# marvinquiet/SpaDOT

Hardware: AMD Instinct MI355X
Metric: training steps/sec + Sinkhorn iters/sec, 50k spots x 3k genes x 5 timepoints (higher is better)
Workload: dtype bf16; 1 GPU; cfg3: 5 time points x 10000 spots x 3000 genes, batch 512, k=30, 1200 inducing points; parallelism=1 GPU, n_sub=9980, E_sub=308893, m_inducing=236, params=16136032, hip_graphs=True, staged_graphs=True, bucketed_grad_exchange=False, units_in_schedule=80

## Files before the change

### spadot_amd/csrc/gemm_bf16.hip

```cpp
#include <hip/hip_runtime.h>
#include <cstdint>

#include "../../include/spadot_model.h"
#include "per_device.h"

#ifndef GEMM_ABLATE
#define GEMM_ABLATE 0
#endif

namespace {

typedef __bf16 bf8 __attribute__((ext_vector_type(8)));
typedef float f16v __attribute__((ext_vector_type(16)));

constexpr int BM = 320, BN = 256, BK = 64, STAGES = 2, NT = 512;
constexpr int ROWB = BK * 2;
constexpr int STAGE_ROWS = BM + BN;
constexpr int STAGEB = STAGE_ROWS * ROWB;
constexpr int PIECES = STAGE_ROWS / 8 / 8;
constexpr int LDS_BYTES = STAGES * STAGEB;

__device__ __forceinline__ unsigned pack2(float lo, float hi) {
    const unsigned short a = __builtin_bit_cast(unsigned short, (__bf16)lo), b = __builtin_bit_cast(unsigned short, (__bf16)hi);
    return (unsigned)a | ((unsigned)b << 16);
}

typedef short s4v __attribute__((ext_vector_type(4)));

template <bool BT>
__global__ __launch_bounds__(NT, 1) void k_gemm_bf16(const __bf16 *__restrict__ A, int lda, const __bf16 *__restrict__ B,
                                                    int ldb, __bf16 *__restrict__ C, int ldc, int M, int N, int K,
                                                    int mtiles, int ntiles, int full_items, int S, int nk_slice,
                                                    float *__restrict__ part, const __bf16 *__restrict__ msk, int ldm, float slope) {
    extern __shared__ __attribute__((aligned(16))) unsigned char smem[];
    const int total = mtiles * ntiles;
    const int full_grid = 8 * ((full_items + 7) >> 3);
    int item, slice = 0;
    if ((int)blockIdx.x < full_grid) {
        const int per_xcd = (full_items + 7) >> 3;
        item = (int)(blockIdx.x & 7) * per_xcd + (int)(blockIdx.x >> 3);
        if (item >= full_items) return;
    } else {
        const int t = (int)blockIdx.x - full_grid;
        item = full_items + t / S;
        slice = t - (t / S) * S;
        if (item >= total) return;
    }
    const bool sliced = item >= full_items;
    const int ks0 = sliced ? slice * nk_slice : 0;
    const int mt = item / ntiles, nt = item - mt * ntiles;
    const int m0 = mt * BM, n0 = nt * BN;
    const int tid = threadIdx.x, lane = tid & 63;
    const int wave = __builtin_amdgcn_readfirstlane(tid >> 6);
    const int wm = wave >> 2, wn = wave & 3;
    const unsigned lds0 = (unsigned)(size_t)smem;

    unsigned off[PIECES];
#pragma unroll
    for (int u = 0; u < PIECES; u++) {
        const int row = 8 * (wave + 8 * u) + (lane >> 3);
        const int chunk = (lane & 7) ^ ((row >> 1) & 7);
        if (u < 5) {
            off[u] = (unsigned)min(m0 + row, M - 1) * (unsigned)(lda * 2) + chunk * 16;
        } else if (!BT) {
            off[u] = (unsigned)(n0 + row - BM) * (unsigned)(ldb * 2) + chunk * 16;
        } else {
            const int brow = 2 * (wave + 8 * (u - 5)) + (lane >> 5);
            off[u] = (unsigned)brow * (unsigned)(ldb * 2) + (unsigned)n0 * 2 + (((lane & 31) ^ ((brow & 3) << 2)) << 4);
        }
    }
    auto request = [&](int ks) __attribute__((always_inline)) {
        const unsigned base = lds0 + (unsigned)(ks % STAGES) * STAGEB + (unsigned)wave * 1024u;
        const char *ga = reinterpret_cast<const char *>(A) + (size_t)(ks0 + ks) * ROWB;
        const char *gb = reinterpret_cast<const char *>(B) + (BT ? (size_t)(ks0 + ks) * BK * ldb * 2 : (size_t)(ks0 + ks) * ROWB);
#pragma unroll
        for (int u = 0; u < PIECES; u++) {
            unsigned keep;
            const unsigned dst = __builtin_amdgcn_readfirstlane(base + (unsigned)u * 8192u);
            asm volatile("s_mov_b32 %0, m0\n\ts_mov_b32 m0, %3\n\ts_nop 0\n\tglobal_load_lds_dwordx4 %1, %2\n\ts_mov_b32 m0, %0"
                         : "=&s"(keep) : "v"(off[u]), "s"(u < 5 ? ga : gb), "s"(dst) : "memory");
        }
    };

    f16v acc[5][2];
#pragma unroll
    for (int i = 0; i < 5; i++)
#pragma unroll
        for (int j = 0; j < 2; j++)
#pragma unroll
            for (int e = 0; e < 16; e++) acc[i][j][e] = 0.f;

    const int r = lane & 31, hh = lane >> 5;
    unsigned a_base[4], b_base[4];
#pragma unroll
    for (int s4 = 0; s4 < 4; s4++) {
        const unsigned sw = (unsigned)(((2 * s4 + hh) ^ ((r >> 1) & 7)) << 4);
        a_base[s4] = lds0 + (unsigned)(wm * 160 + r) * ROWB + sw;
        b_base[s4] = lds0 + (unsigned)(BM + wn * 64 + r) * ROWB + sw;
    }
    unsigned bt_base[2];
    {
        const int g16 = (lane >> 4) & 1, qq = (lane & 15) >> 2, pp = lane & 3;
#pragma unroll
        for (int j = 0; j < 2; j++) {
            const int g = wn * 2 + j;
            bt_base[j] = lds0 + (unsigned)(BM * ROWB) + (unsigned)((8 * hh + qq) * 512 + (g & ~3) * 64 + ((g ^ qq) & 3) * 64 + 32 * g16 + 8 * pp);
        }
    }
    auto read_frags = [&](unsigned stage_off, int s4, bf8 (&af)[5], bf8 (&bf)[2]) __attribute__((always_inline)) {
        if (GEMM_ABLATE & 4) return;
        const unsigned pb = b_base[s4] + stage_off, pa = a_base[s4] + stage_off;
        if (BT) {
#pragma unroll
            for (int j = 0; j < 2; j++) {
                s4v lo, hi;
                const unsigned p = bt_base[j] + stage_off + (unsigned)s4 * 8192u;
                asm volatile("ds_read_b64_tr_b16 %0, %1" : "=v"(lo) : "v"(p));
                asm volatile("ds_read_b64_tr_b16 %0, %1 offset:2048" : "=v"(hi) : "v"(p));
                bf[j] = __builtin_bit_cast(bf8, __builtin_shufflevector(lo, hi, 0, 1, 2, 3, 4, 5, 6, 7));
            }
        } else {
            asm volatile("ds_read_b128 %0, %1" : "=v"(bf[0]) : "v"(pb));
            asm volatile("ds_read_b128 %0, %1 offset:4096" : "=v"(bf[1]) : "v"(pb));
        }
        asm volatile("ds_read_b128 %0, %1" : "=v"(af[0]) : "v"(pa));
        asm volatile("ds_read_b128 %0, %1 offset:4096" : "=v"(af[1]) : "v"(pa));
        asm volatile("ds_read_b128 %0, %1 offset:8192" : "=v"(af[2]) : "v"(pa));
        asm volatile("ds_read_b128 %0, %1 offset:12288" : "=v"(af[3]) : "v"(pa));
        asm volatile("ds_read_b128 %0, %1 offset:16384" : "=v"(af[4]) : "v"(pa));
    };
    auto mma = [&](const bf8 (&af)[5], const bf8 (&bf)[2]) __attribute__((always_inline)) {
        if (GEMM_ABLATE & 2) {
#pragma unroll
            for (int i = 0; i < 5; i++) asm volatile("" ::"v"(af[i]));
#pragma unroll
            for (int j = 0; j < 2; j++) asm volatile("" ::"v"(bf[j]));
            return;
        }
        __builtin_amdgcn_s_setprio(1);
#pragma unroll
        for (int i = 0; i < 5; i++)
#pragma unroll
            for (int j = 0; j < 2; j++) acc[i][j] = __builtin_amdgcn_mfma_f32_32x32x16_bf16(bf[j], af[i], acc[i][j], 0, 0, 0);
        __builtin_amdgcn_s_setprio(0);
    };
    auto frags_ready = [&]() __attribute__((always_inline)) {
        if (BT) asm volatile("s_waitcnt lgkmcnt(9)" ::: "memory");
        else asm volatile("s_waitcnt lgkmcnt(7)" ::: "memory");
        __builtin_amdgcn_sched_barrier(0);
    };

    const int nk = sliced ? min(nk_slice, K / BK - ks0) : K / BK;
    request(0);
    if (1 < nk) {
        request(1);
        asm volatile("s_waitcnt vmcnt(%0)" ::"n"(PIECES) : "memory");
    } else {
        asm volatile("s_waitcnt vmcnt(0)" ::: "memory");
    }
    __builtin_amdgcn_s_barrier();
    bf8 a0[5], b0[2], a1[5], b1[2];
    read_frags(0u, 0, a0, b0);
    for (int P = 0; P < nk; P++) {
        const unsigned so = (unsigned)(P % STAGES) * STAGEB;
        read_frags(so, 1, a1, b1);
        frags_ready();
        mma(a0, b0);
        read_frags(so, 2, a0, b0);
        frags_ready();
        mma(a1, b1);
        read_frags(so, 3, a1, b1);
        frags_ready();
        mma(a0, b0);
        if (P + 1 < nk) {
            asm volatile("s_waitcnt vmcnt(0)" ::: "memory");
            asm volatile("s_waitcnt lgkmcnt(0)" ::: "memory");
            __builtin_amdgcn_sched_barrier(0);
            __builtin_amdgcn_s_barrier();
            if (P + 2 < nk && !(GEMM_ABLATE & 1)) request(P + 2);
            read_frags((unsigned)((P + 1) % STAGES) * STAGEB, 0, a0, b0);
            if (BT) asm volatile("s_waitcnt lgkmcnt(9)" ::: "memory");
            else asm volatile("s_waitcnt lgkmcnt(7)" ::: "memory");
        } else {
            asm volatile("s_waitcnt lgkmcnt(0)" ::: "memory");
        }
        __builtin_amdgcn_sched_barrier(0);
        mma(a1, b1);
    }

    __syncthreads();
    if (sliced) {
        float *tile = part + ((size_t)(item - full_items) * S + slice) * (size_t)(BM * BN);
        unsigned char *patch = smem + (size_t)wave * 8192;
#pragma unroll
        for (int i = 0; i < 5; i++) {
#pragma unroll
            for (int j = 0; j < 2; j++)
#pragma unroll
                for (int g = 0; g < 4; g++) {
                    const int n = j * 32 + 8 * g + 4 * hh;
                    *reinterpret_cast<float4 *>(patch + r * 256 + n * 4) =
                        make_float4(acc[i][j][4 * g], acc[i][j][4 * g + 1], acc[i][j][4 * g + 2], acc[i][j][4 * g + 3]);
                }
            asm volatile("s_waitcnt lgkmcnt(0)" ::: "memory");
#pragma unroll
            for (int p = 0; p < 8; p++) {
                const int pr = p * 4 + (lane >> 4), pc = lane & 15;
                const float4 v = *reinterpret_cast<const float4 *>(patch + pr * 256 + pc * 16);
                *reinterpret_cast<float4 *>(tile + (size_t)(wm * 160 + i * 32 + pr) * BN + wn * 64 + pc * 4) = v;
            }
            asm volatile("s_waitcnt lgkmcnt(0)" ::: "memory");
        }
        return;
    }
    unsigned char *patch = smem + (size_t)wave * 4096;
    typedef unsigned u32x4 __attribute__((ext_vector_type(4)));
    const bool masked = msk != nullptr;
    const __bf16 *mbase = (masked ? msk : C) + n0 + wn * 64 + (lane & 7) * 8;
    const int mld = masked ? ldm : ldc;
    auto mask_row = [&](int i, int p) __attribute__((always_inline)) { return min(m0 + wm * 160 + i * 32 + p * 8 + (lane >> 3), M - 1); };
    u32x4 mkb[2][4];
    if (masked) {
#pragma unroll
        for (int p = 0; p < 4; p++) mkb[0][p] = *reinterpret_cast<const u32x4 *>(mbase + (size_t)mask_row(0, p) * mld);
    }
#pragma unroll
    for (int i = 0; i < 5; i++) {
        if (masked && i + 1 < 5) {
#pragma unroll
            for (int p = 0; p < 4; p++) mkb[(i + 1) & 1][p] = *reinterpret_cast<const u32x4 *>(mbase + (size_t)mask_row(i + 1, p) * mld);
        }
        __builtin_amdgcn_sched_barrier(0);
#pragma unroll
        for (int j = 0; j < 2; j++)
#pragma unroll
            for (int g = 0; g < 4; g++) {
                const int n = j * 32 + 8 * g + 4 * hh;
                *reinterpret_cast<uint2 *>(patch + r * 128 + n * 2) =
                    make_uint2(pack2(acc[i][j][4 * g], acc[i][j][4 * g + 1]), pack2(acc[i][j][4 * g + 2], acc[i][j][4 * g + 3]));
            }
        asm volatile("s_waitcnt lgkmcnt(0)" ::: "memory");
#pragma unroll
        for (int p = 0; p < 4; p++) {
            const int pr = p * 8 + (lane >> 3), pc = lane & 7;
            const int gm = m0 + wm * 160 + i * 32 + pr;
            u32x4 v = *reinterpret_cast<const u32x4 *>(patch + pr * 128 + pc * 16);
            if (masked) {
#pragma unroll
                for (int e = 0; e < 4; e++) {
                    float lo = __uint_as_float(v[e] << 16), hi = __uint_as_float(v[e] & 0xffff0000u);
                    if (!(__uint_as_float(mkb[i & 1][p][e] << 16) > 0.f)) lo *= slope;
                    if (!(__uint_as_float(mkb[i & 1][p][e] & 0xffff0000u) > 0.f)) hi *= slope;
                    v[e] = pack2(lo, hi);
                }
            }
            if (gm < M) *reinterpret_cast<u32x4 *>(C + (size_t)gm * ldc + n0 + wn * 64 + pc * 8) = v;
        }
        asm volatile("s_waitcnt lgkmcnt(0)" ::: "memory");
    }
}

__global__ __launch_bounds__(256) void k_gemm_tail_reduce(const float *__restrict__ part, int S, int ntiles, int first_mt,
                                                         __bf16 *__restrict__ C, int ldc, int M) {
    const int t = blockIdx.x / (BM / 8);
    const int row = (blockIdx.x - t * (BM / 8)) * 8 + (threadIdx.x >> 5), cg = threadIdx.x & 31;
    const int mt = first_mt + t / ntiles, nt = t - (t / ntiles) * ntiles;
    const int gm = mt * BM + row;
    if (gm >= M) return;
    const float *src = part + (size_t)t * S * (size_t)(BM * BN) + (size_t)row * BN + cg * 8;
    float4 a = *reinterpret_cast<const float4 *>(src), b = *reinterpret_cast<const float4 *>(src + 4);
    for (int s_ = 1; s_ < S; s_++) {
        const float4 c = *reinterpret_cast<const float4 *>(src + (size_t)s_ * (BM * BN));
        const float4 d = *reinterpret_cast<const float4 *>(src + (size_t)s_ * (BM * BN) + 4);
        a.x += c.x; a.y += c.y; a.z += c.z; a.w += c.w;
        b.x += d.x; b.y += d.y; b.z += d.z; b.w += d.w;
    }
    *reinterpret_cast<uint4 *>(C + (size_t)gm * ldc + nt * BN + cg * 8) =
        make_uint4(pack2(a.x, a.y), pack2(a.z, a.w), pack2(b.x, b.y), pack2(b.z, b.w));
}

}

template <bool BT>
static int launch_gemm(const void *A, int lda, const void *B, int ldb, void *C, int ldc, int M, int N, int K, void *stream,
                       const void *msk = nullptr, int ldm = 0, float slope = 1.f) {
    if (msk && (ldm < N || ldm % 8 || ((uintptr_t)msk & 15))) return -22;
    if (M <= 0 || N <= 0 || K <= 0 || N % BN != 0 || K % BK != 0 || lda < K || ldb < (BT ? N : K) || ldc < N) return -22;
    if (((uintptr_t)A & 15) || ((uintptr_t)B & 15) || ((uintptr_t)C & 15) || lda % 8 || ldb % 8 || ldc % 8) return -22;
    if ((size_t)M * lda * 2 >= ((size_t)1 << 32) || (size_t)(BT ? K : N) * ldb * 2 >= ((size_t)1 << 32)) return -22;
    static PerDeviceFlag attr_set;     
    if (!attr_set) {
        if (hipFuncSetAttribute((const void *)k_gemm_bf16<BT>, hipFuncAttributeMaxDynamicSharedMemorySize, LDS_BYTES) != hipSuccess) return -5;
        attr_set = true;
    }
    const int mtiles = (M + BM - 1) / BM, ntiles = N / BN;
    const unsigned grid = 8u * (unsigned)((mtiles * ntiles + 7) / 8);
    hipLaunchKernelGGL(k_gemm_bf16<BT>, dim3(grid), dim3(NT), LDS_BYTES, (hipStream_t)stream, (const __bf16 *)A, lda,
                       (const __bf16 *)B, ldb, (__bf16 *)C, ldc, M, N, K, mtiles, ntiles, mtiles * ntiles, 1, K / BK, (float *)nullptr,
                       (const __bf16 *)msk, ldm, slope);
    return hipGetLastError() == hipSuccess ? 0 : -5;
}

extern "C" long long spadot_gemm_bf16_split_workspace(int M, int N, int tail_row_tiles, int slices) {
    if (M <= 0 || N <= 0 || N % BN != 0 || tail_row_tiles < 1 || slices < 2 || slices > 8) return -22;
    const int mtiles = (M + BM - 1) / BM;
    if (tail_row_tiles > mtiles) return -22;
    return (long long)tail_row_tiles * (N / BN) * slices * BM * BN;
}

extern "C" int spadot_gemm_tn_bf16_split(const void *A, int lda, const void *B, int ldb, void *C, int ldc, int M, int N, int K,
                                         int tail_row_tiles, int slices, float *workspace, void *stream) {
    if (M <= 0 || N <= 0 || K <= 0 || N % BN != 0 || K % BK != 0 || lda < K || ldb < K || ldc < N) return -22;
    if (((uintptr_t)A & 15) || ((uintptr_t)B & 15) || ((uintptr_t)C & 15) || lda % 8 || ldb % 8 || ldc % 8) return -22;
    if ((size_t)M * lda * 2 >= ((size_t)1 << 32) || (size_t)N * ldb * 2 >= ((size_t)1 << 32)) return -22;
    const int mtiles = (M + BM - 1) / BM, ntiles = N / BN, nk = K / BK;
    if (tail_row_tiles < 1 || tail_row_tiles > mtiles || slices < 2 || slices > 8 || slices > nk) return -22;
    if (!workspace || ((uintptr_t)workspace & 15)) return -22;
    static PerDeviceFlag attr_set;     
    if (!attr_set) {
        if (hipFuncSetAttribute((const void *)k_gemm_bf16<false>, hipFuncAttributeMaxDynamicSharedMemorySize, LDS_BYTES) != hipSuccess) return -5;
        attr_set = true;
    }
    const int nk_slice = (nk + slices - 1) / slices;
    const int S = (nk + nk_slice - 1) / nk_slice;
    const int full_items = (mtiles - tail_row_tiles) * ntiles, tail_tiles = tail_row_tiles * ntiles;
    const unsigned grid = 8u * (unsigned)((full_items + 7) / 8) + (unsigned)(tail_tiles * S);
    hipLaunchKernelGGL(k_gemm_bf16<false>, dim3(grid), dim3(NT), LDS_BYTES, (hipStream_t)stream, (const __bf16 *)A, lda,
                       (const __bf16 *)B, ldb, (__bf16 *)C, ldc, M, N, K, mtiles, ntiles, full_items, S, nk_slice, workspace,
                       (const __bf16 *)nullptr, 0, 1.f);
    hipLaunchKernelGGL(k_gemm_tail_reduce, dim3((unsigned)(tail_tiles * (BM / 8))), dim3(256), 0, (hipStream_t)stream,
                       (const float *)workspace, S, ntiles, mtiles - tail_row_tiles, (__bf16 *)C, ldc, M);
    return hipGetLastError() == hipSuccess ? 0 : -5;
}

extern "C" int spadot_gemm_tn_bf16(const void *A, int lda, const void *B, int ldb, void *C, int ldc, int M, int N, int K,
                                   void *stream) {
    return launch_gemm<false>(A, lda, B, ldb, C, ldc, M, N, K, stream);
}

extern "C" int spadot_gemm_nn_bf16(const void *A, int lda, const void *B, int ldb, void *C, int ldc, int M, int N, int K,
                                   void *stream) {
    return launch_gemm<true>(A, lda, B, ldb, C, ldc, M, N, K, stream);
}

extern "C" int spadot_gemm_nn_bf16_masked(const void *A, int lda, const void *B, int ldb, void *C, int ldc, int M, int N, int K,
                                          const void *act_out, int ldm, double slope, void *stream) {
    if (!act_out) return -22;
    return launch_gemm<true>(A, lda, B, ldb, C, ldc, M, N, K, stream, act_out, ldm, (float)slope);
}
```

### spadot_amd/csrc/gemm_wgrad_bf16.hip

```cpp
#include <hip/hip_runtime.h>
#include <cstdint>

#include "../../include/spadot_model.h"
#include "per_device.h"

namespace {

typedef __bf16 bf8 __attribute__((ext_vector_type(8)));
typedef short s4v __attribute__((ext_vector_type(4)));
typedef float f16v __attribute__((ext_vector_type(16)));

constexpr int TN = 256, TK = 256, CH = 64, NT = 512;
constexpr int ROWB = 512;
constexpr int OPB = CH * ROWB;
constexpr int STAGEB = 2 * OPB;
constexpr int LDS_BYTES = 2 * STAGEB;
constexpr int PIECES = 8;

template <int WGN, int WGK, int TI, int TJ>
__global__ __launch_bounds__(NT, 1) void k_gemm_wgrad_bf16(const __bf16 *__restrict__ G, int ldg, const __bf16 *__restrict__ X,
                                                          int ldx, float *__restrict__ dW, int ldw, int M, int N, int K,
                                                          int ktiles, int S, int chunks_per_slice,
                                                          const __bf16 *__restrict__ zrow, float *__restrict__ part) {
    extern __shared__ __attribute__((aligned(16))) unsigned char smem[];
    const int tile = blockIdx.x / S, slice = blockIdx.x - tile * S;
    const int tn = tile / ktiles, tk = tile - tn * ktiles;
    static_assert(WGN * WGK == 8 && WGN * TI == 8 && WGK * TJ * 32 <= TK, "wave grid");
    constexpr int TKE = 32 * WGK * TJ;
    constexpr int RD = 2 * (TI + TJ);
    const int n0 = tn * TN, k0 = tk * TKE;
    const int tid = threadIdx.x, lane = tid & 63;
    const int wave = __builtin_amdgcn_readfirstlane(tid >> 6);
    const int wn = wave / WGK, wk = wave - wn * WGK;
    const unsigned lds0 = (unsigned)(size_t)smem;
    const int nchunk_all = (M + CH - 1) / CH;
    const int c_begin = slice * chunks_per_slice, c_end = min(nchunk_all, c_begin + chunks_per_slice);
    const int nk = max(0, c_end - c_begin);

    size_t poff[PIECES];
    int prow[PIECES];
    bool pzero = false;
#pragma unroll
    for (int u = 0; u < PIECES; u++) {
        const int q = wave + 8 * u, qq = q & 31;
        const int row = 2 * qq + (lane >> 5);
        const int chunk = (lane & 31) ^ ((row & 3) << 2);
        prow[u] = row;
        poff[u] = u < 4 ? ((size_t)row * ldg + n0) * 2 + chunk * 16 : ((size_t)row * ldx + k0) * 2 + chunk * 16;
        if (u >= 4 && chunk * 8 >= TKE) pzero = true;
    }
    auto request = [&](int ks) __attribute__((always_inline)) {
#ifdef WGRAD_PROBE_NO_DMA
        return;
#endif
        const int m0 = (c_begin + ks) * CH;
        const unsigned base = lds0 + (unsigned)(ks & 1) * STAGEB + (unsigned)wave * 1024u;
#pragma unroll
        for (int u = 0; u < PIECES; u++) {
            const char *src = (u < 4 ? reinterpret_cast<const char *>(G) + (size_t)m0 * ldg * 2
                                     : reinterpret_cast<const char *>(X) + (size_t)m0 * ldx * 2) + poff[u];
            if (m0 + prow[u] >= M || (u >= 4 && pzero)) src = reinterpret_cast<const char *>(zrow) + (lane & 31) * 16;
            const unsigned dst = __builtin_amdgcn_readfirstlane(base + (unsigned)(u & 3) * 8192u + (u < 4 ? 0u : (unsigned)OPB));
            unsigned keep;
            asm volatile("s_mov_b32 %0, m0\n\ts_mov_b32 m0, %2\n\ts_nop 0\n\tglobal_load_lds_dwordx4 %1, off\n\ts_mov_b32 m0, %0"
                         : "=&s"(keep) : "v"(src), "s"(dst) : "memory");
        }
    };

    f16v acc[TI][TJ];
#pragma unroll
    for (int i = 0; i < TI; i++)
#pragma unroll
        for (int j = 0; j < TJ; j++)
#pragma unroll
            for (int e = 0; e < 16; e++) acc[i][j][e] = 0.f;

    const int hh = lane >> 5, g16 = (lane >> 4) & 1, qq = (lane & 15) >> 2, pp = lane & 3;
    unsigned ga[TI], xb[TJ];
#pragma unroll
    for (int i = 0; i < TI; i++) {
        const int g = wn * TI + i;
        ga[i] = lds0 + (unsigned)((8 * hh + qq) * ROWB + (g & ~3) * 64 + ((g ^ qq) & 3) * 64 + 32 * g16 + 8 * pp);
    }
#pragma unroll
    for (int j = 0; j < TJ; j++) {
        const int g = wk * TJ + j;
        xb[j] = lds0 + (unsigned)OPB + (unsigned)((8 * hh + qq) * ROWB + (g & ~3) * 64 + ((g ^ qq) & 3) * 64 + 32 * g16 + 8 * pp);
    }
    auto read_frags = [&](unsigned stage_off, int ss, s4v (&a)[TI][2], s4v (&b)[TJ][2]) __attribute__((always_inline)) {
        const unsigned so = stage_off + (unsigned)ss * (16 * ROWB);
#ifdef WGRAD_PROBE_NO_READS
#pragma unroll
        for (int j = 0; j < TJ; j++) b[j][0] = b[j][1] = s4v{(short)so, 1, 2, 3};
#pragma unroll
        for (int i = 0; i < TI; i++) a[i][0] = a[i][1] = s4v{(short)so, 1, 2, 3};
        return;
#endif
#pragma unroll
        for (int j = 0; j < TJ; j++) {
            asm volatile("ds_read_b64_tr_b16 %0, %1" : "=v"(b[j][0]) : "v"(xb[j] + so));
            asm volatile("ds_read_b64_tr_b16 %0, %1 offset:2048" : "=v"(b[j][1]) : "v"(xb[j] + so));
        }
#pragma unroll
        for (int i = 0; i < TI; i++) {
            asm volatile("ds_read_b64_tr_b16 %0, %1" : "=v"(a[i][0]) : "v"(ga[i] + so));
            asm volatile("ds_read_b64_tr_b16 %0, %1 offset:2048" : "=v"(a[i][1]) : "v"(ga[i] + so));
        }
    };
    auto mma = [&](const s4v (&a)[TI][2], const s4v (&b)[TJ][2]) __attribute__((always_inline)) {
        __builtin_amdgcn_s_setprio(1);
        bf8 bf[TJ];
#pragma unroll
        for (int j = 0; j < TJ; j++) bf[j] = __builtin_bit_cast(bf8, __builtin_shufflevector(b[j][0], b[j][1], 0, 1, 2, 3, 4, 5, 6, 7));
#pragma unroll
        for (int i = 0; i < TI; i++) {
            const bf8 af = __builtin_bit_cast(bf8, __builtin_shufflevector(a[i][0], a[i][1], 0, 1, 2, 3, 4, 5, 6, 7));
#pragma unroll
            for (int j = 0; j < TJ; j++) {
#ifdef WGRAD_PROBE_NO_MFMA
                asm volatile("" ::"v"(af), "v"(bf[j]));
#else
                acc[i][j] = __builtin_amdgcn_mfma_f32_32x32x16_bf16(af, bf[j], acc[i][j], 0, 0, 0);
#endif
            }
        }
        __builtin_amdgcn_s_setprio(0);
    };
    auto frags_ready = [&]() __attribute__((always_inline)) {
#ifdef WGRAD_PROBE_NO_READS
        return;
#endif
        asm volatile("s_waitcnt lgkmcnt(%0)" ::"n"(RD) : "memory");
        __builtin_amdgcn_sched_barrier(0);
    };

    if (nk > 0) {
        request(0);
        if (1 < nk) {
            request(1);
            asm volatile("s_waitcnt vmcnt(%0)" ::"n"(PIECES) : "memory");
        } else {
            asm volatile("s_waitcnt vmcnt(0)" ::: "memory");
        }
        __builtin_amdgcn_s_barrier();
        s4v a0[TI][2], b0[TJ][2], a1[TI][2], b1[TJ][2];
        read_frags(0u, 0, a0, b0);
        for (int P = 0; P < nk; P++) {
            const unsigned so = (unsigned)(P & 1) * STAGEB;
            read_frags(so, 1, a1, b1);
            frags_ready();
            mma(a0, b0);
            read_frags(so, 2, a0, b0);
            frags_ready();
            mma(a1, b1);
            read_frags(so, 3, a1, b1);
            frags_ready();
            mma(a0, b0);
            if (P + 1 < nk) {
                asm volatile("s_waitcnt vmcnt(0)" ::: "memory");
                asm volatile("s_waitcnt lgkmcnt(0)" ::: "memory");
                __builtin_amdgcn_sched_barrier(0);
                __builtin_amdgcn_s_barrier();
                if (P + 2 < nk) request(P + 2);
                read_frags((unsigned)((P + 1) & 1) * STAGEB, 0, a0, b0);
                asm volatile("s_waitcnt lgkmcnt(%0)" ::"n"(RD) : "memory");
            } else {
                asm volatile("s_waitcnt lgkmcnt(0)" ::: "memory");
            }
            __builtin_amdgcn_sched_barrier(0);
            mma(a1, b1);
        }
    }

    const int lk = (wk * TJ) * 32 + (lane & 31);
    if (S == 1) {
#pragma unroll
        for (int i = 0; i < TI; i++)
#pragma unroll
            for (int j = 0; j < TJ; j++)
#pragma unroll
                for (int e = 0; e < 16; e++) {
                    const int n = n0 + (wn * TI + i) * 32 + (e & 3) + 8 * (e >> 2) + 4 * hh, k = k0 + lk + 32 * j;
                    if (n < N && k < K) dW[(size_t)n * ldw + k] = acc[i][j][e];
                }
        return;
    }
    float *mine = part + ((size_t)slice * gridDim.x / S + tile) * (size_t)(TN * TKE);
#pragma unroll
    for (int i = 0; i < TI; i++)
#pragma unroll
        for (int j = 0; j < TJ; j++)
#pragma unroll
            for (int e = 0; e < 16; e++) {
                const int ln = (wn * TI + i) * 32 + (e & 3) + 8 * (e >> 2) + 4 * hh;
                mine[(size_t)ln * TKE + lk + 32 * j] = acc[i][j][e];
            }
}

template <int TKE>
__global__ __launch_bounds__(256) void k_wgrad_reduce(const float *__restrict__ part, int S, int tiles, int ktiles,
                                                      float *__restrict__ dW, int ldw, int N, int K) {
    constexpr int RP = TKE / 4;
    constexpr int BPT = RP / 4;
    constexpr int Q = 64 * RP;
    typedef float f32x4 __attribute__((ext_vector_type(4)));
    const int tile = blockIdx.x / BPT;
    const int p0 = (blockIdx.x - tile * BPT) * 256 + threadIdx.x;
    const int tn = tile / ktiles, tk = tile - tn * ktiles;
    f32x4 v[8][4];
#pragma unroll
    for (int s_ = 0; s_ < 8; s_++)
        if (s_ < S) {
            const f32x4 *src = reinterpret_cast<const f32x4 *>(part + ((size_t)s_ * tiles + tile) * (size_t)(TN * TKE));
#pragma unroll
            for (int j = 0; j < 4; j++) v[s_][j] = src[p0 + j * Q];
        }
#pragma unroll
    for (int j = 0; j < 4; j++) {
        f32x4 sum = v[0][j];
#pragma unroll
        for (int s_ = 1; s_ < 8; s_++)
            if (s_ < S) sum += v[s_][j];
        const int idx4 = p0 + j * Q, ln = idx4 / RP, c4 = idx4 - ln * RP;
        const int n = tn * TN + ln, k = tk * TKE + 4 * c4;
        if (n < N && k + 3 < K) *reinterpret_cast<f32x4 *>(dW + (size_t)n * ldw + k) = sum;
        else if (n < N) {
            for (int e = 0; e < 4; e++)
                if (k + e < K) dW[(size_t)n * ldw + k + e] = sum[e];
        }
    }
}

static int effective_slices(int M, int slices, int *cps_out) {
    const int nchunk = (M + CH - 1) / CH;
    int S = slices > 0 ? slices : 1;
    if (S > nchunk) S = nchunk;
    if (S > 8) S = 8;
    const int cps = (nchunk + S - 1) / S;
    S = (nchunk + cps - 1) / cps;
    if (cps_out) *cps_out = cps;
    return S;
}

}

extern "C" long long spadot_gemm_wgrad_bf16_workspace_tiled(int M, int N, int K, int slices, int tile_k) {
    if (M <= 0 || N <= 0 || K <= 0 || N % TN != 0 || (tile_k != 256 && tile_k != 192)) return -22;
    const int S = effective_slices(M, slices, nullptr);
    const long long tiles = (long long)(N / TN) * ((K + tile_k - 1) / tile_k);
    return S > 1 ? (long long)S * tiles * TN * tile_k : 0;
}

extern "C" long long spadot_gemm_wgrad_bf16_workspace(int M, int N, int K, int slices) {
    return spadot_gemm_wgrad_bf16_workspace_tiled(M, N, K, slices, 256);
}

template <int WGN, int WGK, int TI, int TJ>
static int launch_wgrad(const void *G, int ldg, const void *X, int ldx, float *dW, int ldw, int M, int N, int K, int ktiles, int ntiles,
                        int S, int cps, float *workspace, const void *zero_row, hipStream_t stream) {
    constexpr int TKE = 32 * WGK * TJ;
    static PerDeviceFlag attr_set;     
    auto kern = k_gemm_wgrad_bf16<WGN, WGK, TI, TJ>;
    if (!attr_set) {
        if (hipFuncSetAttribute((const void *)kern, hipFuncAttributeMaxDynamicSharedMemorySize, LDS_BYTES) != hipSuccess) return -5;
        attr_set = true;
    }
    const int tiles = ntiles * ktiles;
    hipLaunchKernelGGL(kern, dim3((unsigned)(tiles * S)), dim3(NT), LDS_BYTES, stream, (const __bf16 *)G, ldg, (const __bf16 *)X, ldx, dW,
                       ldw, M, N, K, ktiles, S, cps, (const __bf16 *)zero_row, workspace);
    if (S > 1)
        hipLaunchKernelGGL(k_wgrad_reduce<TKE>, dim3((unsigned)tiles * (unsigned)(TKE / 16)), dim3(256), 0, stream, (const float *)workspace, S,
                           tiles, ktiles, dW, ldw, N, K);
    return hipGetLastError() == hipSuccess ? 0 : -5;
}

extern "C" int spadot_gemm_wgrad_bf16_tiled(const void *G, int ldg, const void *X, int ldx, float *dW, int ldw, int M, int N, int K,
                                            int slices, int tile_k, float *workspace, const void *zero_row, void *stream) {
    if (M <= 0 || N <= 0 || K <= 0 || N % TN != 0 || ldg < N || ldx < K || ldw < K || ldg % 8 || ldx % 8) return -22;
    if (tile_k != 256 && tile_k != 192) return -22;
    if (((uintptr_t)G & 15) || ((uintptr_t)X & 15) || ((uintptr_t)dW & 15) || (ldw % 4)) return -22;
    if (!zero_row || ((uintptr_t)zero_row & 15)) return -22;
    const int ktiles = (K + tile_k - 1) / tile_k, ntiles = N / TN;
    if (ldx < ktiles * tile_k) return -22;
    if ((size_t)M * ldg * 2 >= ((size_t)1 << 32) || (size_t)M * ldx * 2 >= ((size_t)1 << 32)) return -22;
    int cps = 0;
    const int S = effective_slices(M, slices, &cps);
    if (ntiles * ktiles > 4096) return -22;
    if (S > 1 && (!workspace || ((uintptr_t)workspace & 15))) return -22;
    if (tile_k == 256)
        return launch_wgrad<2, 4, 4, 2>(G, ldg, X, ldx, dW, ldw, M, N, K, ktiles, ntiles, S, cps, workspace, zero_row, (hipStream_t)stream);
    return launch_wgrad<4, 2, 2, 3>(G, ldg, X, ldx, dW, ldw, M, N, K, ktiles, ntiles, S, cps, workspace, zero_row, (hipStream_t)stream);
}

extern "C" int spadot_gemm_wgrad_bf16(const void *G, int ldg, const void *X, int ldx, float *dW, int ldw, int M, int N, int K,
                                      int slices, float *workspace, const void *zero_row, void *stream) {
    return spadot_gemm_wgrad_bf16_tiled(G, ldg, X, ldx, dW, ldw, M, N, K, slices, 256, workspace, zero_row, stream);
}
```

Baseline: 671.5 training steps/s.

## Switch GEMM and wgrad kernels to 16x16x32 MFMA tiles by default

Adds a compile-time switch that replaces the 32x32x16 bf16 MFMA with the 16x16x32 variant in both the forward/dgrad GEMM and the weight-gradient kernel, and makes it the default. Fragment loads, LDS swizzles for the transposed B operand, the accumulator layout and the epilogue patch writers are all reworked for 16x16 tiles, with the MMA split into halves interleaved with LDS reads. The aim is better instruction issue and overlap of LDS reads with MFMA work. In exchange it issues more MFMA instructions and more LDS reads per tile, and the new swizzle and output index maps carry correctness risk.

```diff
diff --git a/spadot_amd/csrc/gemm_bf16.hip b/spadot_amd/csrc/gemm_bf16.hip
--- a/spadot_amd/csrc/gemm_bf16.hip
+++ b/spadot_amd/csrc/gemm_bf16.hip
@@ -7,11 +7,18 @@
 #ifndef GEMM_ABLATE
 #define GEMM_ABLATE 0
 #endif
+#ifndef GEMM_MFMA_SHAPE
+#define GEMM_MFMA_SHAPE 16
+#endif
+#if GEMM_MFMA_SHAPE != 16 && GEMM_MFMA_SHAPE != 32
+#error "GEMM_MFMA_SHAPE is 16 or 32"
+#endif
 
 namespace {
 
 typedef __bf16 bf8 __attribute__((ext_vector_type(8)));
 typedef float f16v __attribute__((ext_vector_type(16)));
+typedef float f4v __attribute__((ext_vector_type(4)));
 
 constexpr int BM = 320, BN = 256, BK = 64, STAGES = 2, NT = 512;
 constexpr int ROWB = BK * 2;
@@ -66,7 +73,8 @@
             off[u] = (unsigned)(n0 + row - BM) * (unsigned)(ldb * 2) + chunk * 16;
         } else {
             const int brow = 2 * (wave + 8 * (u - 5)) + (lane >> 5);
-            off[u] = (unsigned)brow * (unsigned)(ldb * 2) + (unsigned)n0 * 2 + (((lane & 31) ^ ((brow & 3) << 2)) << 4);
+            const int bsw = ((brow & 3) << 2) | (GEMM_MFMA_SHAPE == 16 ? ((brow >> 3) & 1) << 1 : 0);
+            off[u] = (unsigned)brow * (unsigned)(ldb * 2) + (unsigned)n0 * 2 + (((lane & 31) ^ bsw) << 4);
         }
     }
     auto request = [&](int ks) __attribute__((always_inline)) {
@@ -82,6 +90,141 @@
         }
     };
 
+    const int nk = sliced ? min(nk_slice, K / BK - ks0) : K / BK;
+    auto prologue = [&]() __attribute__((always_inline)) {
+        request(0);
+        if (1 < nk) {
+            request(1);
+            asm volatile("s_waitcnt vmcnt(%0)" ::"n"(PIECES) : "memory");
+        } else {
+            asm volatile("s_waitcnt vmcnt(0)" ::: "memory");
+        }
+        __builtin_amdgcn_s_barrier();
+    };
+
+#if GEMM_MFMA_SHAPE == 16
+    f4v acc[10][4];
+#pragma unroll
+    for (int i = 0; i < 10; i++)
+#pragma unroll
+        for (int j = 0; j < 4; j++)
+#pragma unroll
+            for (int e = 0; e < 4; e++) acc[i][j][e] = 0.f;
+
+    const int r = lane & 15, q4 = lane >> 4;
+    unsigned a_base[2], b_base[2];
+#pragma unroll
+    for (int s2 = 0; s2 < 2; s2++) {
+        const unsigned sw = (unsigned)(((4 * s2 + q4) ^ ((r >> 1) & 7)) << 4);
+        a_base[s2] = lds0 + (unsigned)(wm * 160 + r) * ROWB + sw;
+        b_base[s2] = lds0 + (unsigned)(BM + wn * 64 + r) * ROWB + sw;
+    }
+    unsigned bt_base[4];
+    {
+        const int qq = (lane & 15) >> 2, pp = lane & 3;
+#pragma unroll
+        for (int jt = 0; jt < 4; jt++) {
+            const int c = (4 * (2 * wn + (jt >> 1)) + 2 * (jt & 1) + (pp >> 1)) ^ (qq << 2) ^ ((q4 & 1) << 1);
+            bt_base[jt] = lds0 + (unsigned)(BM * ROWB) + (unsigned)((8 * q4 + qq) * 512 + c * 16 + 8 * (pp & 1));
+        }
+    }
+    constexpr int B_READS = BT ? 8 : 4;
+    auto read_b = [&](unsigned stage_off, int s2, bf8 (&bf)[4]) __attribute__((always_inline)) {
+        if (GEMM_ABLATE & 4) return;
+        if (BT) {
+#pragma unroll
+            for (int jt = 0; jt < 4; jt++) {
+                s4v lo, hi;
+                const unsigned p = bt_base[jt] + stage_off + (unsigned)s2 * 16384u;
+                asm volatile("ds_read_b64_tr_b16 %0, %1" : "=v"(lo) : "v"(p));
+                asm volatile("ds_read_b64_tr_b16 %0, %1 offset:2048" : "=v"(hi) : "v"(p));
+                bf[jt] = __builtin_bit_cast(bf8, __builtin_shufflevector(lo, hi, 0, 1, 2, 3, 4, 5, 6, 7));
+            }
+        } else {
+            const unsigned pb = b_base[s2] + stage_off;
+            asm volatile("ds_read_b128 %0, %1" : "=v"(bf[0]) : "v"(pb));
+            asm volatile("ds_read_b128 %0, %1 offset:2048" : "=v"(bf[1]) : "v"(pb));
+            asm volatile("ds_read_b128 %0, %1 offset:4096" : "=v"(bf[2]) : "v"(pb));
+            asm volatile("ds_read_b128 %0, %1 offset:6144" : "=v"(bf[3]) : "v"(pb));
+        }
+    };
+    auto read_a = [&](unsigned stage_off, int s2, int h, bf8 (&af)[5]) __attribute__((always_inline)) {
+        if (GEMM_ABLATE & 4) return;
+        const unsigned pa = a_base[s2] + stage_off + (unsigned)h * (80u * ROWB);
+        asm volatile("ds_read_b128 %0, %1" : "=v"(af[0]) : "v"(pa));
+        asm volatile("ds_read_b128 %0, %1 offset:2048" : "=v"(af[1]) : "v"(pa));
+        asm volatile("ds_read_b128 %0, %1 offset:4096" : "=v"(af[2]) : "v"(pa));
+        asm volatile("ds_read_b128 %0, %1 offset:6144" : "=v"(af[3]) : "v"(pa));
+        asm volatile("ds_read_b128 %0, %1 offset:8192" : "=v"(af[4]) : "v"(pa));
+    };
+#define GEMM_MMA_HALF(H, AF, BF)                                                                                              \
+    {                                                                                                                         \
+        if (GEMM_ABLATE & 2) {                                                                                                \
+            _Pragma("unroll") for (int i = 0; i < 5; i++) asm volatile("" ::"v"(AF[i]));                                      \
+            _Pragma("unroll") for (int j = 0; j < 4; j++) asm volatile("" ::"v"(BF[j]));                                      \
+        } else {                                                                                                              \
+            __builtin_amdgcn_s_setprio(1);                                                                                    \
+            _Pragma("unroll") for (int i = 0; i < 5; i++)                                                                     \
+                _Pragma("unroll") for (int j = 0; j < 4; j++)                                                                 \
+                    acc[5 * (H) + i][j] = __builtin_amdgcn_mfma_f32_16x16x32_bf16(BF[j], AF[i], acc[5 * (H) + i][j], 0, 0, 0); \
+            __builtin_amdgcn_s_setprio(0);                                                                                    \
+        }                                                                                                                     \
+    }
+#define GEMM_FRAGS_READY(n)                                  \
+    {                                                        \
+        asm volatile("s_waitcnt lgkmcnt(%0)" ::"n"(n) : "memory"); \
+        __builtin_amdgcn_sched_barrier(0);                   \
+    }
+
+    prologue();
+    bf8 ax[5], ay[5], ba[4], bb[4];
+    read_b(0u, 0, ba);
+    read_a(0u, 0, 0, ax);
+    for (int P = 0; P < nk; P++) {
+        const unsigned so = (unsigned)(P % STAGES) * STAGEB;
+        read_a(so, 0, 1, ay);
+        GEMM_FRAGS_READY(5);
+        GEMM_MMA_HALF(0, ax, ba);
+        read_b(so, 1, bb);
+        read_a(so, 1, 0, ax);
+        GEMM_FRAGS_READY(B_READS + 5);
+        GEMM_MMA_HALF(1, ay, ba);
+        read_a(so, 1, 1, ay);
+        GEMM_FRAGS_READY(5);
+        GEMM_MMA_HALF(0, ax, bb);
+        if (P + 1 < nk) {
+            asm volatile("s_waitcnt vmcnt(0)" ::: "memory");
+            asm volatile("s_waitcnt lgkmcnt(0)" ::: "memory");
+            __builtin_amdgcn_sched_barrier(0);
+            __builtin_amdgcn_s_barrier();
+            if (P + 2 < nk && !(GEMM_ABLATE & 1)) request(P + 2);
+            read_b((unsigned)((P + 1) % STAGES) * STAGEB, 0, ba);
+            read_a((unsigned)((P + 1) % STAGES) * STAGEB, 0, 0, ax);
+        } else {
+            asm volatile("s_waitcnt lgkmcnt(0)" ::: "memory");
+        }
+        __builtin_amdgcn_sched_barrier(0);
+        GEMM_MMA_HALF(1, ay, bb);
+    }
+#undef GEMM_MMA_HALF
+#undef GEMM_FRAGS_READY
+    auto patch_f32 = [&](unsigned char *patch, int i) __attribute__((always_inline)) {
+#pragma unroll
+        for (int t = 0; t < 2; t++)
+#pragma unroll
+            for (int j = 0; j < 4; j++)
+                *reinterpret_cast<float4 *>(patch + (16 * t + r) * 256 + (16 * j + 4 * q4) * 4) =
+                    make_float4(acc[2 * i + t][j][0], acc[2 * i + t][j][1], acc[2 * i + t][j][2], acc[2 * i + t][j][3]);
+    };
+    auto patch_bf16 = [&](unsigned char *patch, int i) __attribute__((always_inline)) {
+#pragma unroll
+        for (int t = 0; t < 2; t++)
+#pragma unroll
+            for (int j = 0; j < 4; j++)
+                *reinterpret_cast<uint2 *>(patch + (16 * t + r) * 128 + (16 * j + 4 * q4) * 2) =
+                    make_uint2(pack2(acc[2 * i + t][j][0], acc[2 * i + t][j][1]), pack2(acc[2 * i + t][j][2], acc[2 * i + t][j][3]));
+    };
+#else
     f16v acc[5][2];
 #pragma unroll
     for (int i = 0; i < 5; i++)
@@ -150,15 +293,7 @@
         __builtin_amdgcn_sched_barrier(0);
     };
 
-    const int nk = sliced ? min(nk_slice, K / BK - ks0) : K / BK;
-    request(0);
-    if (1 < nk) {
-        request(1);
-        asm volatile("s_waitcnt vmcnt(%0)" ::"n"(PIECES) : "memory");
-    } else {
-        asm volatile("s_waitcnt vmcnt(0)" ::: "memory");
-    }
-    __builtin_amdgcn_s_barrier();
+    prologue();
     bf8 a0[5], b0[2], a1[5], b1[2];
     read_frags(0u, 0, a0, b0);
     for (int P = 0; P < nk; P++) {
@@ -188,20 +323,35 @@
         mma(a1, b1);
     }
 
+    auto patch_f32 = [&](unsigned char *patch, int i) __attribute__((always_inline)) {
+#pragma unroll
+        for (int j = 0; j < 2; j++)
+#pragma unroll
+            for (int g = 0; g < 4; g++) {
+                const int n = j * 32 + 8 * g + 4 * hh;
+                *reinterpret_cast<float4 *>(patch + r * 256 + n * 4) =
+                    make_float4(acc[i][j][4 * g], acc[i][j][4 * g + 1], acc[i][j][4 * g + 2], acc[i][j][4 * g + 3]);
+            }
+    };
+    auto patch_bf16 = [&](unsigned char *patch, int i) __attribute__((always_inline)) {
+#pragma unroll
+        for (int j = 0; j < 2; j++)
+#pragma unroll
+            for (int g = 0; g < 4; g++) {
+                const int n = j * 32 + 8 * g + 4 * hh;
+                *reinterpret_cast<uint2 *>(patch + r * 128 + n * 2) =
+                    make_uint2(pack2(acc[i][j][4 * g], acc[i][j][4 * g + 1]), pack2(acc[i][j][4 * g + 2], acc[i][j][4 * g + 3]));
+            }
+    };
+#endif
+
     __syncthreads();
     if (sliced) {
         float *tile = part + ((size_t)(item - full_items) * S + slice) * (size_t)(BM * BN);
         unsigned char *patch = smem + (size_t)wave * 8192;
 #pragma unroll
         for (int i = 0; i < 5; i++) {
-#pragma unroll
-            for (int j = 0; j < 2; j++)
-#pragma unroll
-                for (int g = 0; g < 4; g++) {
-                    const int n = j * 32 + 8 * g + 4 * hh;
-                    *reinterpret_cast<float4 *>(patch + r * 256 + n * 4) =
-                        make_float4(acc[i][j][4 * g], acc[i][j][4 * g + 1], acc[i][j][4 * g + 2], acc[i][j][4 * g + 3]);
-                }
+            patch_f32(patch, i);
             asm volatile("s_waitcnt lgkmcnt(0)" ::: "memory");
 #pragma unroll
             for (int p = 0; p < 8; p++) {
@@ -231,14 +381,7 @@
             for (int p = 0; p < 4; p++) mkb[(i + 1) & 1][p] = *reinterpret_cast<const u32x4 *>(mbase + (size_t)mask_row(i + 1, p) * mld);
         }
         __builtin_amdgcn_sched_barrier(0);
-#pragma unroll
-        for (int j = 0; j < 2; j++)
-#pragma unroll
-            for (int g = 0; g < 4; g++) {
-                const int n = j * 32 + 8 * g + 4 * hh;
-                *reinterpret_cast<uint2 *>(patch + r * 128 + n * 2) =
-                    make_uint2(pack2(acc[i][j][4 * g], acc[i][j][4 * g + 1]), pack2(acc[i][j][4 * g + 2], acc[i][j][4 * g + 3]));
-            }
+        patch_bf16(patch, i);
         asm volatile("s_waitcnt lgkmcnt(0)" ::: "memory");
 #pragma unroll
         for (int p = 0; p < 4; p++) {
diff --git a/spadot_amd/csrc/gemm_wgrad_bf16.hip b/spadot_amd/csrc/gemm_wgrad_bf16.hip
--- a/spadot_amd/csrc/gemm_wgrad_bf16.hip
+++ b/spadot_amd/csrc/gemm_wgrad_bf16.hip
@@ -3,12 +3,20 @@
 
 #include "../../include/spadot_model.h"
 #include "per_device.h"
+
+#ifndef WGRAD_MFMA_SHAPE
+#define WGRAD_MFMA_SHAPE 16
+#endif
+#if WGRAD_MFMA_SHAPE != 16 && WGRAD_MFMA_SHAPE != 32
+#error "WGRAD_MFMA_SHAPE is 16 or 32"
+#endif
 
 namespace {
 
 typedef __bf16 bf8 __attribute__((ext_vector_type(8)));
 typedef short s4v __attribute__((ext_vector_type(4)));
 typedef float f16v __attribute__((ext_vector_type(16)));
+typedef float f4v __attribute__((ext_vector_type(4)));
 
 constexpr int TN = 256, TK = 256, CH = 64, NT = 512;
 constexpr int ROWB = 512;
@@ -44,7 +52,7 @@
     for (int u = 0; u < PIECES; u++) {
         const int q = wave + 8 * u, qq = q & 31;
         const int row = 2 * qq + (lane >> 5);
-        const int chunk = (lane & 31) ^ ((row & 3) << 2);
+        const int chunk = (lane & 31) ^ ((row & 3) << 2) ^ (WGRAD_MFMA_SHAPE == 16 ? ((row >> 3) & 1) << 1 : 0);
         prow[u] = row;
         poff[u] = u < 4 ? ((size_t)row * ldg + n0) * 2 + chunk * 16 : ((size_t)row * ldx + k0) * 2 + chunk * 16;
         if (u >= 4 && chunk * 8 >= TKE) pzero = true;
@@ -67,6 +75,130 @@
         }
     };
 
+#if WGRAD_MFMA_SHAPE == 16
+    constexpr int TI2 = 2 * TI, TJ2 = 2 * TJ;
+    f4v acc[TI2][TJ2];
+#pragma unroll
+    for (int i = 0; i < TI2; i++)
+#pragma unroll
+        for (int j = 0; j < TJ2; j++)
+#pragma unroll
+            for (int e = 0; e < 4; e++) acc[i][j][e] = 0.f;
+
+    const int q4 = lane >> 4, qq = (lane & 15) >> 2, pp = lane & 3;
+    auto image = [&](int t) __attribute__((always_inline)) {
+        const int c = (2 * t + (pp >> 1)) ^ (qq << 2) ^ ((q4 & 1) << 1);
+        return (unsigned)((8 * q4 + qq) * ROWB + c * 16 + 8 * (pp & 1));
+    };
+    unsigned ga[TI2], xb[TJ2];
+#pragma unroll
+    for (int i = 0; i < TI2; i++) ga[i] = lds0 + image(wn * TI2 + i);
+#pragma unroll
+    for (int j = 0; j < TJ2; j++) xb[j] = lds0 + (unsigned)OPB + image(wk * TJ2 + j);
+    constexpr int RA = 2 * TI, RB = 2 * TJ2;
+    auto read_b = [&](unsigned stage_off, int s2, s4v (&b)[TJ2][2]) __attribute__((always_inline)) {
+        const unsigned so = stage_off + (unsigned)s2 * (32 * ROWB);
+#pragma unroll
+        for (int j = 0; j < TJ2; j++) {
+            asm volatile("ds_read_b64_tr_b16 %0, %1" : "=v"(b[j][0]) : "v"(xb[j] + so));
+            asm volatile("ds_read_b64_tr_b16 %0, %1 offset:2048" : "=v"(b[j][1]) : "v"(xb[j] + so));
+        }
+    };
+#define WGRAD_READ_A(STAGE_OFF, S2, H, A)                                                                      \
+    {                                                                                                          \
+        const unsigned so_ = (STAGE_OFF) + (unsigned)(S2) * (32 * ROWB);                                       \
+        _Pragma("unroll") for (int i = 0; i < TI; i++) {                                                       \
+            asm volatile("ds_read_b64_tr_b16 %0, %1" : "=v"(A[i][0]) : "v"(ga[(H) * TI + i] + so_));           \
+            asm volatile("ds_read_b64_tr_b16 %0, %1 offset:2048" : "=v"(A[i][1]) : "v"(ga[(H) * TI + i] + so_)); \
+        }                                                                                                      \
+    }
+#define WGRAD_MMA_HALF(H, A, B)                                                                                \
+    {                                                                                                          \
+        __builtin_amdgcn_s_setprio(1);                                                                         \
+        bf8 bf_[TJ2];                                                                                          \
+        _Pragma("unroll") for (int j = 0; j < TJ2; j++)                                                        \
+            bf_[j] = __builtin_bit_cast(bf8, __builtin_shufflevector(B[j][0], B[j][1], 0, 1, 2, 3, 4, 5, 6, 7)); \
+        _Pragma("unroll") for (int i = 0; i < TI; i++) {                                                       \
+            const bf8 af_ = __builtin_bit_cast(bf8, __builtin_shufflevector(A[i][0], A[i][1], 0, 1, 2, 3, 4, 5, 6, 7)); \
+            _Pragma("unroll") for (int j = 0; j < TJ2; j++)                                                    \
+                acc[(H) * TI + i][j] = __builtin_amdgcn_mfma_f32_16x16x32_bf16(af_, bf_[j], acc[(H) * TI + i][j], 0, 0, 0); \
+        }                                                                                                      \
+        __builtin_amdgcn_s_setprio(0);                                                                         \
+    }
+#define WGRAD_FRAGS_READY(n)                                        \
+    {                                                               \
+        asm volatile("s_waitcnt lgkmcnt(%0)" ::"n"(n) : "memory"); \
+        __builtin_amdgcn_sched_barrier(0);                          \
+    }
+
+    if (nk > 0) {
+        request(0);
+        if (1 < nk) {
+            request(1);
+            asm volatile("s_waitcnt vmcnt(%0)" ::"n"(PIECES) : "memory");
+        } else {
+            asm volatile("s_waitcnt vmcnt(0)" ::: "memory");
+        }
+        __builtin_amdgcn_s_barrier();
+        s4v ax[TI][2], ay[TI][2], ba[TJ2][2], bb[TJ2][2];
+        read_b(0u, 0, ba);
+        WGRAD_READ_A(0u, 0, 0, ax);
+        for (int P = 0; P < nk; P++) {
+            const unsigned so = (unsigned)(P & 1) * STAGEB;
+            WGRAD_READ_A(so, 0, 1, ay);
+            WGRAD_FRAGS_READY(RA);
+            WGRAD_MMA_HALF(0, ax, ba);
+            read_b(so, 1, bb);
+            WGRAD_FRAGS_READY(RB);
+            WGRAD_READ_A(so, 1, 0, ax);
+            WGRAD_MMA_HALF(1, ay, ba);
+            WGRAD_READ_A(so, 1, 1, ay);
+            WGRAD_FRAGS_READY(RA);
+            WGRAD_MMA_HALF(0, ax, bb);
+            if (P + 1 < nk) {
+                asm volatile("s_waitcnt vmcnt(0)" ::: "memory");
+                asm volatile("s_waitcnt lgkmcnt(0)" ::: "memory");
+                __builtin_amdgcn_sched_barrier(0);
+                __builtin_amdgcn_s_barrier();
+                if (P + 2 < nk) request(P + 2);
+                read_b((unsigned)((P + 1) & 1) * STAGEB, 0, ba);
+                WGRAD_READ_A((unsigned)((P + 1) & 1) * STAGEB, 0, 0, ax);
+            } else {
+                asm volatile("s_waitcnt lgkmcnt(0)" ::: "memory");
+            }
+            __builtin_amdgcn_sched_barrier(0);
+            WGRAD_MMA_HALF(1, ay, bb);
+        }
+    }
+#undef WGRAD_READ_A
+#undef WGRAD_MMA_HALF
+#undef WGRAD_FRAGS_READY
+
+    const int lk = (wk * TJ2) * 16 + (lane & 15);
+    if (S == 1) {
+#pragma unroll
+        for (int i = 0; i < TI2; i++)
+#pragma unroll
+            for (int j = 0; j < TJ2; j++)
+#pragma unroll
+                for (int e = 0; e < 4; e++) {
+                    const int n = n0 + (wn * TI2 + i) * 16 + 4 * q4 + e, k = k0 + lk + 16 * j;
+                    if (n < N && k < K) dW[(size_t)n * ldw + k] = acc[i][j][e];
+                }
+        return;
+    }
+    float *mine = part + ((size_t)slice * gridDim.x / S + tile) * (size_t)(TN * TKE);
+#pragma unroll
+    for (int i = 0; i < TI2; i++)
+#pragma unroll
+        for (int j = 0; j < TJ2; j++)
+#pragma unroll
+            for (int e = 0; e < 4; e++) {
+                const int ln = (wn * TI2 + i) * 16 + 4 * q4 + e;
+                mine[(size_t)ln * TKE + lk + 16 * j] = acc[i][j][e];
+            }
+}
+#else
     f16v acc[TI][TJ];
 #pragma unroll
     for (int i = 0; i < TI; i++)
@@ -196,6 +328,7 @@
                 mine[(size_t)ln * TKE + lk + 32 * j] = acc[i][j][e];
             }
 }
+#endif
 
 template <int TKE>
 __global__ __launch_bounds__(256) void k_wgrad_reduce(const float *__restrict__ part, int S, int tiles, int ktiles,
```

Measured after the change: 678.1 training steps/s, median of 6. Within noise of the previous version (+1.0%).
